# kishwarshafin/pepper

Hardware: AMD Instinct MI355X
Metric: inference windows/sec (whole node) (higher is better)
Workload: dtype f32 via f16 hi/lo split operands (3 MFMAs per product), f32 accumulate

## Files before the change

pepper_amd/csrc/api.hip:

```cpp
#include "../../include/pepper_amd.h"

#include <hip/hip_runtime.h>

#include <algorithm>
#include <cmath>
#include <cstdio>
#include <cstdlib>
#include <cstring>
#include <map>
#include <string>
#include <vector>

#include "dec_frag16.h"
#include "kernels.h"

namespace {
thread_local std::string g_err;
}

namespace pa {
int set_error(int code, const std::string& msg) {
    g_err = msg;
    return code;
}
// ... 496 lines not shown
    if (!as_base(m)) return fail(PA_ERR_INVALID, "bad model handle");
    if (on != 0 && on != 1) return fail(PA_ERR_INVALID, std::string(entry) + ": on must be 0 or 1");
    m->batch_invariant = on != 0;
    return PA_OK;
}

template <class M>
int get_batch_invariant(M* m, int32_t* on) {
    if (!as_base(m) || !on) return fail(PA_ERR_INVALID, "bad model handle");
    *on = m->batch_invariant ? 1 : 0;
    return PA_OK;
}

enum Proj { IN_LOOP, XP_GEMM_H2, XP_GEMM_F32 };
template <class Rec>
struct LayerForm {
    Proj proj;
    Rec rec;
    bool y_h2;
};

}

struct pa_variant_model : ModelBase {
    pa_variant_config cfg{};
    int H = 256, L1 = 512;
    bool split_gemm = true;
    bool split_rec = true;
    int64_t small_batch = 3072;
    int64_t small_rows = 3072;
    std::vector<RecLayer> rec;
    Linear lin[5], out;
    DevBuf *mlp_w = nullptr, *mlp_b = nullptr;
    DevBuf *mlp_w32 = nullptr;
    int* ovf_counter() const {
        return mlp_w32 ? reinterpret_cast<int*>(static_cast<char*>(mlp_w32->p) + 4 * sizeof(float*)) : nullptr;
    }
    DevBuf *xp, *ya, *yb, *l1, *l2, *stage_in[2], *stage_p[2], *stage_l[2];
    bool unit_split = true;
    int split_holdoff = 0;
    int64_t split_fallbacks = 0;
    int split_sabotage = 0;
    DevBuf *us_exch = nullptr, *us_cnt = nullptr, *us_failed = nullptr;
    int* us_host = nullptr;
    bool batch_invariant = false;
    ~pa_variant_model() override {
        if (us_host) (void)hipHostFree(us_host);
    }
};

extern "C" {

const char* pa_last_error(void) { return g_err.c_str(); }
const char* pa_version(void) { return "pepper_amd 0.1.0 gfx950"; }
int pa_device_count(void) {
    int c = 0;
    if (hipGetDeviceCount(&c) != hipSuccess) return 0;
    return c;
}

int pa_variant_create(const pa_variant_config* cfg, const char* const* names, const float* const* data,
                      const int64_t* numel, int32_t n_tensors, void* hip_stream, pa_variant_model** out) {
    if (!cfg || !names || !data || !numel || !out) return fail(PA_ERR_INVALID, "null argument");
    if (cfg->image_features <= 0 || cfg->window <= 0 || cfg->gru_layers <= 0 ||
        cfg->num_classes_type <= 0 || cfg->num_classes_type > 8)
        return fail(PA_ERR_INVALID, "bad pa_variant_config");
    auto* m = new pa_variant_model();
    m->cfg = *cfg;
    const int H = m->H;
    StateDict sd(names, data, numel, n_tensors);
    int rc = create_common(m, sd, cfg->window, H, hip_stream);
    if (const char* e = getenv("PA_SMALL_BATCH")) m->small_batch = atoll(e);
    if (const char* e = getenv("PA_SMALL_ROWS")) m->small_rows = atoll(e);
    if (const char* e = getenv("PA_UNIT_SPLIT")) m->unit_split = e[0] != '0';
    if (const char* e = getenv("PA_UNIT_SPLIT_SABOTAGE")) m->split_sabotage = atoi(e);
    for (int mod = 0; mod < 2 && rc == PA_OK; ++mod)
        for (int layer = 0; layer < cfg->gru_layers && rc == PA_OK; ++layer) {
            const int K = (mod == 0 && layer == 0) ? cfg->image_features : 2 * H;
            m->rec.emplace_back();
            rc = build_rec_layer(m, sd, mod == 0 ? "encoder" : "decoder", layer, 4, H, K, m->rec.back(), m->split_rec,
                                 m->split_gemm);
        }
    const char* lin_names[5] = {"linear_1", "linear_2", "linear_3", "linear_4", "linear_5"};
    for (int i = 0; i < 5 && rc == PA_OK; ++i)
        rc = build_linear(m, sd, lin_names[i], i == 0 ? 2 * H * cfg->window : m->L1, m->L1, m->lin[i],
                          i == 0 && m->split_gemm);
    if (rc == PA_OK) rc = build_linear(m, sd, "output_layer_type", m->L1, cfg->num_classes_type, m->out);
    if (rc == PA_OK && m->split_gemm && m->L1 == 512) {
        std::string err;
        const float* w4[4];
        std::vector<float> b4((size_t)4 * m->L1);
        bool ok = true;
        for (int i = 0; i < 4 && ok; ++i) {
            w4[i] = sd.get(std::string(lin_names[i + 1]) + ".weight", (int64_t)m->L1 * m->L1, err);
            const float* b = sd.get(std::string(lin_names[i + 1]) + ".bias", m->L1, err);
            ok = fits_f16(w4[i], (int64_t)m->L1 * m->L1);
            std::memcpy(&b4[(size_t)i * m->L1], b, m->L1 * sizeof(float));
        }
        if (ok) {
            std::vector<uint32_t> packed(pa::mlp_weights_h2_words(4));
            float scale[4];
            pa::pack_mlp_weights_h2(w4, 4, packed.data(), scale);
            std::vector<float> table((size_t)8 * m->L1 + 4);
            for (int i = 0; i < 4; ++i) {
                for (int k = 0; k < m->L1; ++k) {
                    table[(size_t)i * m->L1 + k] = b4[(size_t)i * m->L1 + k] * scale[i];
                    table[(size_t)4 * m->L1 + 4 + (size_t)i * m->L1 + k] = b4[(size_t)i * m->L1 + k];
                }
// ... 126 lines not shown
            LAUNCH_TRY(m, "lstm_rec_fused_in", 2.0 * n * T * (4.0 * H) * (H + r.K) * 2,
                       pa::launch_lstm_rec_fused(H, static_cast<const int8_t*>(cur), r.K, r.b_in->f(),
                                                 r.w_cat->f(), y, 2 * H, (int)n, T, m->stream));
            break;
        case FUSED_DEC_H2:
            LAUNCH_TRY(m, "lstm_dec_h2_fused", 2.0 * n * T * (4.0 * H) * (H + r.K) * 2,
                       pa::launch_lstm_dec_h2(H, cur, cur_ld, bias_l, r.w_cat_dec_h2->p, y, 2 * H, (int)n, T, m->stream,
                                              bi && s.small_rows));
            break;
        case SPLIT_H2: {
            const int sabotage = m->split_sabotage > 0 ? 1 : 0;
            m->split_sabotage -= sabotage;
            LAUNCH_TRY(m, "lstm_rec_h2_split", 2.0 * n * T * (4.0 * H) * H * 2,
                       pa::launch_lstm_rec_h2_split(H, m->xp->f(), NX, r.w_hh_h2->p, y, 2 * H, (int)n, T, m->us_exch->p,
                                                    m->us_cnt->p, static_cast<int*>(m->us_failed->p), m->stream, sabotage));
            break;
        }
        case PLAIN_H2:
            LAUNCH_TRY(m, "lstm_rec_h2", 2.0 * n * T * (4.0 * H) * H * 2,
                       pa::launch_lstm_seed_h2(H, m->xp->f(), NX, r.w_hh_h2->p, y, 2 * H, (int)n, T, m->stream, s.small_rows));
            break;
        case PLAIN_F32:
            LAUNCH_TRY(m, "lstm_rec", 2.0 * n * T * (4.0 * H) * H * 2,
                       pa::launch_lstm_rec(H, m->xp->f(), NX, r.w_hh->f(), y, 2 * H, (int)n, T, m->stream));
            break;
        }
        cur = y;
        cur_kind = pa::A_F32;
        cur_ld = 2 * H;
        cur_h2 = f.y_h2;
        which ^= 1;
    }
    const int K1 = T * 2 * H;
    if (m->split_gemm && m->lin[0].w_h2 != nullptr && cur_kind == pa::A_F32) {
        if (!cur_h2)
            LAUNCH_TRY(m, "cvt_h2", 0.0,
                       pa::launch_f32_to_h2(static_cast<const float*>(cur), const_cast<void*>(cur), n, K1, K1, m->stream));
        LAUNCH_TRY(m, "gemm_h2_linear_1", 2.0 * n * m->L1 * K1,
                   pa::launch_gemm_h2(cur, K1, (size_t)n * K1 * 4, m->lin[0].w_h2->p, K1, (size_t)m->L1 * K1 * 4,
                                      m->lin[0].b->f(), m->l1->f(), m->L1, (int)n, m->L1, K1, 1, 0, 0, 0, 0, m->stream,
                                      s.l1_splits > 1 ? m->xp->f() : nullptr, s.l1_splits));
    } else {
        LAUNCH_TRY(m, "gemm_linear_1", 2.0 * n * m->L1 * K1,
                   pa::launch_gemm_nt(pa::A_F32, cur, K1, m->lin[0].w->f(), K1, m->lin[0].b->f(), m->l1->f(),
                                      m->L1, (int)n, m->L1, K1, 1, 0, 0, 0, 0, m->stream));
    }
    if (m->mlp_w != nullptr && C <= 8) {
        LAUNCH_TRY(m, "mlp_tail_h2", 2.0 * n * m->L1 * (4.0 * m->L1 + C),
                   pa::launch_mlp_tail_h2(m->l1->f(), m->L1, m->mlp_w->p, m->mlp_b->f(), 4, m->out.w->f(), m->out.b->f(), C,
                                          probs, logits, (int)n, m->stream, static_cast<const float* const*>(m->mlp_w32->p),
                                          ovf_counter, bi));
        if (s.unit_split) {
            HIP_TRY(hipMemcpyAsync(&m->us_host[0], m->us_failed->p, sizeof(int), hipMemcpyDeviceToHost, m->stream));
            HIP_TRY(hipStreamSynchronize(m->stream));
            if (m->us_host[0] != 0) {
                ++m->split_fallbacks;
                m->split_holdoff = US_HOLDOFF;
                HIP_TRY(hipMemcpyAsync(ovf_counter, &m->us_host[1], sizeof(int), hipMemcpyHostToDevice, m->stream));
                return variant_forward_chunk(m, a_kind, images, n, probs, logits, false);
            }
        }
        return PA_OK;
    }
    float* a = m->l1->f();
    float* b = m->l2->f();
    for (int i = 1; i < 5; ++i) {
        LAUNCH_TRY(m, "gemm_linear_2to5", 2.0 * n * m->L1 * m->L1,
                   pa::launch_gemm_nt(pa::A_F32, a, m->L1, m->lin[i].w->f(), m->L1, m->lin[i].b->f(), b,
                                      m->L1, (int)n, m->L1, m->L1, 1, 0, 0, 0, 0, m->stream));
        std::swap(a, b);
    }
    LAUNCH_TRY(m, "head_softmax", 2.0 * n * m->L1 * C,
               pa::launch_dense_small(0, a, m->L1, m->out.w->f(), m->out.b->f(), probs, logits, (int)n,
                                      m->L1, C, 1, 1, 0, m->stream));
    return PA_OK;
}

static int variant_forward(pa_variant_model* m, int a_kind, const void* images, size_t elem, int64_t n,
                           float* probs, float* logits) {
    if (!as_base(m)) return fail(PA_ERR_INVALID, "bad model handle");
    if (n < 0 || (n > 0 && (!images || !probs))) return fail(PA_ERR_INVALID, "null buffer");
    HIP_TRY(hipSetDevice(m->device));
    const int64_t per = (int64_t)m->cfg.window * m->cfg.image_features;
    const int C = m->cfg.num_classes_type;
// ... 478 lines not shown
```

pepper_amd/csrc/gemm_h2.hip:

```cpp
#include "common.h"
#include "kernels.h"

#include <cstdlib>
#include <vector>

namespace {

typedef _Float16 h8 __attribute__((ext_vector_type(8)));

constexpr int HM = 256, HN = 256, HK = 32;
constexpr int HROW = 36;
constexpr int HSTAGE = (HM + HN) * HROW;

PA_DEV f32x16 mfma_h(h8 a, h8 b, f32x16 c) { return __builtin_amdgcn_mfma_f32_32x32x16_f16(a, b, c, 0, 0, 0); }

template <int ACT, int EXP = 0>
__global__ __launch_bounds__(256) void gemm_h2_kernel(const uint32_t* __restrict__ A, int lda, uint32_t a_bytes,
                                                      const uint32_t* __restrict__ W, int ldw, uint32_t w_bytes,
                                                      const float* __restrict__ bias, float* __restrict__ C, int ldc,
                                                      int M, int N, int K, int tiles_n, int nwg, int a_rpb,
                                                      int64_t a_bstride, int frag_T, int frag_nb) {
    __shared__ __attribute__((aligned(16))) uint32_t lds[2 * HSTAGE];

    const int tile = xcd_swizzle(blockIdx.x, nwg);
// ... 348 lines not shown
}

namespace pa {

static bool g_h2_split_parent = false;
int g_h2_exp = 0;

void split_h2_host(const float* src, uint32_t* dst, int64_t rows, int K, int64_t ld_src, int64_t ld_dst) {
    for (int64_t r = 0; r < rows; ++r) {
        const float* s = src + r * ld_src;
        _Float16* d = reinterpret_cast<_Float16*>(dst + r * ld_dst);
        for (int g = 0; g < K / 8; ++g)
            for (int e = 0; e < 8; ++e) {
                const float v = s[g * 8 + e];
                const _Float16 hi = (_Float16)v;
                d[g * 16 + e] = hi;
                d[g * 16 + 8 + e] = (_Float16)(v - (float)hi);
            }
    }
}

hipError_t launch_f32_to_h2(const float* src, void* dst, int64_t rows, int K, int64_t ld, hipStream_t stream) {
    if ((K & 7) || (ld & 7)) return hipErrorInvalidValue;
    const int64_t n = rows * (K >> 3);
    if (n == 0) return hipSuccess;
    hipLaunchKernelGGL(f32_to_h2_kernel, dim3((unsigned)((n + 255) / 256)), dim3(256), 0, stream, src,
                       reinterpret_cast<uint32_t*>(dst), rows, K, ld);
    return hipGetLastError();
}

hipError_t launch_gemm_h2(const void* A, int lda, size_t a_bytes, const void* W, int ldw, size_t w_bytes,
                          const float* bias, float* C, int ldc, int M, int N, int K, int act, int a_rpb,
                          int64_t a_bstride, int frag_T, int frag_nb, hipStream_t stream, float* splitk_ws,
                          int splits) {
    if (frag_T > 0 && ((M & 31) || (N & 31) || act != 0)) return hipErrorInvalidValue;
    if ((K % HK) || (lda & 7) || (ldw & 7) || (a_bstride & 7) || ((uintptr_t)A & 15) || ((uintptr_t)W & 15))
        return hipErrorInvalidValue;
    if (a_bytes >= (1ull << 32) || w_bytes >= (1ull << 32)) return hipErrorInvalidValue;
    const int tiles_m = (M + HM - 1) / HM, tiles_n = (N + HN - 1) / HN;
    const int nwg = tiles_m * tiles_n;
    if (nwg == 0) return hipSuccess;
    const uint32_t* Au = reinterpret_cast<const uint32_t*>(A);
    const uint32_t* Wu = reinterpret_cast<const uint32_t*>(W);
    if (splits > 1 && splitk_ws != nullptr && frag_T == 0 && !(N & 3) && K / HK >= splits) {
        if (g_h2_split_parent)
            hipLaunchKernelGGL((gemm_h2_kernel<0>), dim3(nwg, splits), dim3(256), 0, stream, Au, lda, (uint32_t)a_bytes, Wu,
                               ldw, (uint32_t)w_bytes, (const float*)nullptr, splitk_ws, N, M, N, K, tiles_n, nwg, a_rpb,
                               a_bstride, 0, 0);
        else
            hipLaunchKernelGGL(gemm_h2_k32_kernel, dim3(nwg, splits), dim3(256), 0, stream, Au, lda, (uint32_t)a_bytes, Wu,
                               ldw, (uint32_t)w_bytes, splitk_ws, M, N, K, tiles_n, nwg, a_rpb, a_bstride);
        const size_t n4 = (size_t)M * (N >> 2);
        if (act == 1)
            hipLaunchKernelGGL((splitk_finish_kernel<1>), dim3((unsigned)((n4 + 255) / 256)), dim3(256), 0, stream,
                               splitk_ws, splits, bias, C, ldc, M, N);
        else
            hipLaunchKernelGGL((splitk_finish_kernel<0>), dim3((unsigned)((n4 + 255) / 256)), dim3(256), 0, stream,
                               splitk_ws, splits, bias, C, ldc, M, N);
        return hipGetLastError();
    }
    if (g_h2_exp > 0 && g_h2_exp < 8) {
#define PA_EXP(E_) case E_: hipLaunchKernelGGL((gemm_h2_kernel<0, E_>), dim3(nwg), dim3(256), 0, stream, Au, lda, (uint32_t)a_bytes, Wu, ldw, (uint32_t)w_bytes, bias, C, ldc, M, N, K, tiles_n, nwg, a_rpb, a_bstride, frag_T, frag_nb); break;
        switch (g_h2_exp) { PA_EXP(1) PA_EXP(2) PA_EXP(3) PA_EXP(4) PA_EXP(5) PA_EXP(6) PA_EXP(7) }
#undef PA_EXP
        return hipGetLastError();
    }
    if (act == 1)
        hipLaunchKernelGGL((gemm_h2_kernel<1>), dim3(nwg), dim3(256), 0, stream, Au, lda, (uint32_t)a_bytes, Wu, ldw,
                           (uint32_t)w_bytes, bias, C, ldc, M, N, K, tiles_n, nwg, a_rpb, a_bstride, frag_T, frag_nb);
    else
        hipLaunchKernelGGL((gemm_h2_kernel<0>), dim3(nwg), dim3(256), 0, stream, Au, lda, (uint32_t)a_bytes, Wu, ldw,
                           (uint32_t)w_bytes, bias, C, ldc, M, N, K, tiles_n, nwg, a_rpb, a_bstride, frag_T, frag_nb);
    return hipGetLastError();
}

}

extern "C" void pa_debug_gemm_h2_experiment(int e) { pa::g_h2_exp = e; }

extern "C" int pa_debug_gemm_h2(const float* A, const float* W, const float* bias, float* C, int a_rows, int M, int N,
                                int K, int act, int frag_T, int frag_nb, int iters, float* ms_out) {
    void *dA = nullptr, *dA2 = nullptr, *dW = nullptr, *dB = nullptr, *dC = nullptr;
    const size_t a_bytes = (size_t)a_rows * K * 4, w_bytes = (size_t)N * K * 4;
    const size_t c_elems = frag_T > 0 ? (size_t)M * N : (size_t)M * N;
// ... 83 lines not shown
```

pepper_amd/csrc/kernels.h:

```cpp
#pragma once
#include <hip/hip_runtime.h>
#include <stdint.h>

#include <string>

namespace pa {

int set_error(int code, const std::string& msg);

enum AKind { A_F32 = 0, A_I8 = 1, A_U8 = 2, A_F32_SCALAR = 3 };

hipError_t launch_gemm_nt(int a_type, const void* A, int lda, const float* W, int ldw,
                          const float* bias, float* C, int ldc, int M, int N, int K, int act,
                          int a_rpb, int64_t a_bstride, int frag_T, int frag_nb, hipStream_t stream);

hipError_t launch_gemm_h2(const void* A, int lda, size_t a_bytes, const void* W, int ldw, size_t w_bytes,
                          const float* bias, float* C, int ldc, int M, int N, int K, int act, int a_rpb,
                          int64_t a_bstride, int frag_T, int frag_nb, hipStream_t stream,
                          float* splitk_ws = nullptr, int splits = 1);
hipError_t launch_f32_to_h2(const float* src, void* dst, int64_t rows, int K, int64_t ld, hipStream_t stream);
void split_h2_host(const float* src, uint32_t* dst, int64_t rows, int K, int64_t ld_src, int64_t ld_dst);

hipError_t launch_lstm_rec(int H, const float* Xp, int ldx, const float* Wp, float* Y, int ldy,
                           int B, int T, hipStream_t stream);
hipError_t launch_lstm_rec_fused(int H, const int8_t* X, int F, const float* bias, const float* Wcat,
                                 float* Y, int ldy, int B, int T, hipStream_t stream);
hipError_t launch_gru_rec(int H, const float* Xp, int ldx, const float* Wp, const float* bhn,
                          const float* h0, int ldh0, float* hn, int ldhn, float* Y, int ldy,
                          int B, int T, hipStream_t stream);

hipError_t launch_gru_rec_fused(int H, const uint8_t* X, int F, int64_t x_bstride, const float* bias,
                                const float* Wcat, const float* bhn, const float* h0, int ldh0, float* hn, int ldhn,
                                float* Y, int ldy, int B, int T, hipStream_t stream);

void pack_rec_weights_h2(const float* const whh[2], const float* const wih[2], int G, int H, int F, int KX,
                         uint32_t* out, const float* const* bias = nullptr);
size_t rec_weights_h2_words(int G, int H, int KX);
int gru_fused_input_kx(int H, int F);
hipError_t launch_lstm_seed_h2(int H, const float* Xp, int ldx, const void* Wp, void* Y, int ldy, int B, int T,
                               hipStream_t stream, bool small = false);
hipError_t launch_lstm_enc_h2(int H, const int8_t* X, int F, const float* bias, const void* Wp, void* Y, int ldy, int B, int T,
                              hipStream_t stream, bool small = false);

size_t lstm_split_exchange_bytes(int B);
size_t lstm_split_counter_bytes(int B);
int lstm_split_grid(int B);
int lstm_split_resident_workgroups(int ntw);
hipError_t launch_lstm_rec_h2_split(int H, const float* Xp, int ldx, const void* Wp, void* Y, int ldy, int B, int T, void* exch,
                                    void* counters, int* failed, hipStream_t stream, int sabotage = 0);

hipError_t launch_lstm_dec_h2(int H, const void* Xh, int ldxh, const float* bias, const void* Wp, void* Y, int ldy, int B,
                              int T, hipStream_t stream, bool small = false);
hipError_t launch_gru_rec_h2(int H, const float* Xp, int ldx, const uint8_t* X, int F, int64_t x_bstride,
                             const float* bias, const void* Wp, const float* bhn, const float* h0, int ldh0, float* hn,
                             int ldhn, void* Y, int ldy, int B, int T, hipStream_t stream);

void pack_gru_small_weights_h2(const float* const whh[2], int H, uint32_t* out);
size_t gru_small_weights_h2_words(int H);
hipError_t launch_gru_small_h2(int H, const float* Xp, int ldx, const void* Wp, const float* bhn, const float* h0, int ldh0,
                               float* hn, int ldhn, void* Y, int ldy, int B, int T, hipStream_t stream);
hipError_t launch_gru_dec_h2(int H, const void* Xh, int ldxh, const float* bias, const void* Wp, const float* bhn,
                             const float* h0, int ldh0, float* hn, int ldhn, void* Y, int ldy, int B, int T,
                             hipStream_t stream);

void pack_dense_head_h2(const float* W, int C, int H, uint32_t* out);
size_t dense_head_h2_words(int H);
size_t dense_partials_floats(int B, int T);
hipError_t launch_gru_dec_h2_dense(int H, const void* Xh, int ldxh, const float* bias, const void* Wp, const float* bhn,
                                   const float* h0, int ldh0, float* hn, int ldhn, const void* Wd, float* P, int B, int T,
                                   hipStream_t stream);
hipError_t launch_polish_combine(const float* P, const float* bias, float* acc, int B, int T, int C, int S, int off,
                                 hipStream_t stream);

void pack_mlp_weights_h2(const float* const* W, int NL, uint32_t* out, float* scale);
size_t mlp_weights_h2_words(int NL);
hipError_t launch_mlp_tail_h2(const float* X, int ldx, const void* Wp, const float* bias, int NL, const float* Wout,
                              const float* bout, int C, float* probs, float* logits, int n, hipStream_t stream,
                              const float* const* W32, int* overflow_rows, bool per_row = false);

hipError_t launch_dense_small(int mode, const float* X, int ldx, const float* W, const float* bias,
                              float* out0, float* out1, int rows, int K, int C, int T, int S, int off,
                              hipStream_t stream);
hipError_t launch_polish_dense_acc_h2(const void* X, int ldx, const float* W, const float* bias, float* acc, int rows,
                                      int K, int C, int T, int S, int off, hipStream_t stream);
hipError_t launch_h2_to_f32(void* buf, int64_t rows, int K, int64_t ld, hipStream_t stream);
hipError_t launch_polish_finalize(const float* acc, uint8_t* labels, uint8_t* phred, int64_t B, int S,
                                  int C, int overlap, hipStream_t stream);

void launch_bgzf_inflate(hipStream_t stream, const uint8_t* comp, const int64_t* comp_off, const int32_t* comp_len,
                         const int64_t* out_off, const int32_t* out_len, uint8_t* out, int32_t* status, int n_blocks,
                         int64_t comp_bytes, unsigned long long* debug_counts = nullptr);
const char* inflate_status_text(int32_t s);
void launch_record_walk(hipStream_t stream, const uint8_t* data, int64_t data_bytes, const int64_t* entries, int n_entries, int cap,
                        void* slots, int32_t* counts, int32_t* base, int32_t* flags, void* out, int64_t out_cap, int32_t* tail,
                        int split = 0);
}
```

pepper_amd/csrc/mlp_h2.hip:

```cpp
#include "common.h"
#include "kernels.h"

namespace {

typedef _Float16 h8 __attribute__((ext_vector_type(8)));

constexpr int MT = 64, D = 512, KS = D / 16, NTILES = D / 32;
constexpr int ROWB = D * 4 + 16, ROWD = ROWB / 4;

PA_DEV f32x16 mfma_h(h8 a, h8 b, f32x16 c) { return __builtin_amdgcn_mfma_f32_32x32x16_f16(a, b, c, 0, 0, 0); }

template <int NL, bool PERROW = false>
__global__ __launch_bounds__(512, 1) void mlp_tail_h2_kernel(const float* __restrict__ X, int ldx,
                                                             const uint32_t* __restrict__ Wp,
                                                             const float* __restrict__ bias,
                                                             const float* __restrict__ Wout,
                                                             const float* __restrict__ bout, int C,
                                                             float* __restrict__ probs, float* __restrict__ logits,
                                                             int n, const float* const* __restrict__ W32,
                                                             int* __restrict__ overflow_rows) {
    extern __shared__ __attribute__((aligned(16))) uint32_t lds[];
    static_assert((ROWB / 16) % 2 == 1, "row stride must be an odd number of 16-byte slots");
    const int tid = threadIdx.x, lane = tid & 63;
    const int w = __builtin_amdgcn_readfirstlane(tid >> 6);
    const int li = lane & 31, hf = lane >> 5;
    const int b0 = blockIdx.x * MT;

    bool bad = false;
    uint32_t* rowbad = lds + MT * ROWD;
    {
        const int row = tid >> 3, gsel = tid & 7;
        int grow = b0 + row;
        grow = grow < n ? grow : n - 1;
        const float* src = X + (size_t)grow * ldx;
#pragma unroll
        for (int j = 0; j < 8; ++j) {
            const int g = gsel + 8 * j;
            const f32x4 a = *reinterpret_cast<const f32x4*>(src + g * 8);
            const f32x4 b = *reinterpret_cast<const f32x4*>(src + g * 8 + 4);
            const float v[8] = {a.x, a.y, a.z, a.w, b.x, b.y, b.z, b.w};
            h8 hi, lo;
#pragma unroll
            for (int e = 0; e < 8; ++e) {
                bad |= !(fabsf(v[e]) < 65504.0f);
                hi[e] = (_Float16)v[e];
                lo[e] = (_Float16)(v[e] - (float)hi[e]);
            }
            *reinterpret_cast<h8*>(lds + row * ROWD + g * 8) = hi;
            *reinterpret_cast<h8*>(lds + row * ROWD + g * 8 + 4) = lo;
        }
        if (PERROW) {
            int b8 = bad ? 1 : 0;
            b8 |= __shfl_xor(b8, 1, 64);
            b8 |= __shfl_xor(b8, 2, 64);
            b8 |= __shfl_xor(b8, 4, 64);
            if (gsel == 0) rowbad[row] = (uint32_t)b8;
        }
    }
    __syncthreads();

    const uint32_t* arow = lds + li * ROWD + hf * 8;
    const bool odd = li & 1;
    struct Frag { h8 b[2][2], a[2][2]; };

#pragma unroll 1
    for (int layer = 0; layer < NL; ++layer) {
        const __amdgpu_buffer_rsrc_t wrs = __builtin_amdgcn_make_buffer_rsrc(
            const_cast<uint32_t*>(Wp + ((size_t)layer * NTILES + 2 * w) * KS * 512), 0, 0x7fffffff, 0x00020000);
        const unsigned woff = lane * 16u;
        auto load_step = [&](int s, Frag& fr) {
#pragma unroll
            for (int nn = 0; nn < 2; ++nn)
#pragma unroll
                for (int hl = 0; hl < 2; ++hl)
                    fr.b[nn][hl] = __builtin_bit_cast(h8, __builtin_amdgcn_raw_buffer_load_b128(
                                                              wrs, woff, (unsigned)((nn * KS + s) * 2 + hl) * 1024u, 0));
#pragma unroll
            for (int m = 0; m < 2; ++m) {
                fr.a[m][0] = *reinterpret_cast<const h8*>(arow + m * 32 * ROWD + s * 16);
                fr.a[m][1] = *reinterpret_cast<const h8*>(arow + m * 32 * ROWD + s * 16 + 4);
            }
        };
        f32x16 acc[2][2];
#pragma unroll
        for (int nn = 0; nn < 2; ++nn) {
            const float bv = bias[layer * D + 64 * w + 32 * nn + li];
#pragma unroll
            for (int m = 0; m < 2; ++m)
#pragma unroll
                for (int r = 0; r < 16; ++r) acc[m][nn][r] = bv;
        }
        Frag ring[2];
        load_step(0, ring[0]);
#pragma unroll
        for (int s = 0; s < KS; ++s) {
            const int p = s & 1;
            if (s + 1 < KS) load_step(s + 1, ring[p ^ 1]);
#pragma unroll
            for (int term = 0; term < 3; ++term)
#pragma unroll
                for (int nn = 0; nn < 2; ++nn)
#pragma unroll
                    for (int m = 0; m < 2; ++m)
                        acc[m][nn] = mfma_h(ring[p].a[m][term == 0 ? 1 : 0], ring[p].b[nn][term == 1 ? 1 : 0], acc[m][nn]);
            if (s + 1 < KS) {
#pragma unroll
                for (int q = 0; q < 4; ++q) {
                    __builtin_amdgcn_sched_group_barrier(0x008, 1, 0);
                    __builtin_amdgcn_sched_group_barrier(0x020, 1, 0);
                }
#pragma unroll
                for (int q = 0; q < 4; ++q) {
                    __builtin_amdgcn_sched_group_barrier(0x008, 1, 0);
                    __builtin_amdgcn_sched_group_barrier(0x100, 1, 0);
                }
                __builtin_amdgcn_sched_group_barrier(0x008, 4, 0);
            }
            __builtin_amdgcn_sched_barrier(0);
        }
        lds_barrier();
        const float unscale = bias[NL * D + layer];
#pragma unroll
        for (int nn = 0; nn < 2; ++nn) {
            const int col = 64 * w + 32 * nn + li;
            uint32_t* dst = lds + 4 * hf * ROWD + (col >> 3) * 8 + (odd ? 4 : 0) + ((col & 7) >> 1);
#pragma unroll
            for (int m = 0; m < 2; ++m)
#pragma unroll
                for (int r = 0; r < 16; ++r) {
                    const float v = selu_f(acc[m][nn][r] * unscale);
                    bad |= !(fabsf(v) < 65504.0f);
                    if (PERROW && !(fabsf(v) < 65504.0f)) rowbad[4 * hf + 32 * m + (r & 3) + 8 * (r >> 2)] = 1u;
                    dst[(32 * m + (r & 3) + 8 * (r >> 2)) * ROWD] = h2_word_of(v, h2_select(odd));
                }
        }
        lds_barrier();
    }

    float* frow = reinterpret_cast<float*>(lds);
    auto head = [&](bool from_f32, bool select) {
        float wo[8][8];
#pragma unroll
        for (int c = 0; c < 8; ++c)
#pragma unroll
            for (int e = 0; e < 8; ++e) wo[c][e] = c < C ? Wout[(size_t)c * D + lane * 8 + e] : 0.0f;
        for (int rr = 0; rr < 8; ++rr) {
            const int row = 8 * w + rr;
            if (PERROW && select && (rowbad[row] != 0) != from_f32) continue;
            const h8 hi = *reinterpret_cast<const h8*>(lds + row * ROWD + lane * 8);
            const h8 lo = *reinterpret_cast<const h8*>(lds + row * ROWD + lane * 8 + 4);
            float x[8];
#pragma unroll
            for (int e = 0; e < 8; ++e) x[e] = from_f32 ? frow[row * ROWD + lane * 8 + e] : (float)hi[e] + (float)lo[e];
            float logit[8], mx = -INFINITY;
#pragma unroll
            for (int c = 0; c < 8; ++c) {
                float p = 0.0f;
#pragma unroll
                for (int e = 0; e < 8; ++e) p += x[e] * wo[c][e];
#pragma unroll
                for (int o = 32; o > 0; o >>= 1) p += __shfl_xor(p, o, 64);
                logit[c] = c < C ? p + bout[c < C ? c : 0] : -INFINITY;
                mx = fmaxf(mx, logit[c]);
            }
            float e[8], den = 0.0f;
#pragma unroll
            for (int c = 0; c < 8; ++c) {
                e[c] = c < C ? expf(logit[c] - mx) : 0.0f;
                den += e[c];
            }
            float my_logit = 0.0f, my_e = 0.0f;
#pragma unroll
            for (int c = 0; c < 8; ++c)
                if (lane == c) { my_logit = logit[c]; my_e = e[c]; }
            const int grow = b0 + row;
            if (grow < n && lane < C) {
                probs[(size_t)grow * C + lane] = my_e / den;
                if (logits != nullptr) logits[(size_t)grow * C + lane] = my_logit;
            }
        }
    };

    const bool rerun = __syncthreads_or(bad ? 1 : 0) != 0;
    if (PERROW) {
        head(false, rerun);
        if (rerun) __syncthreads();
    }
    if (rerun) {
        if (tid == 0 && overflow_rows != nullptr) {
            int cnt = n - b0 < MT ? n - b0 : MT;
            if (PERROW) {
                cnt = 0;
                for (int r = 0; r < MT && b0 + r < n; ++r) cnt += rowbad[r] != 0 ? 1 : 0;
            }
            atomicAdd(overflow_rows, cnt);
        }
        for (int i = tid; i < MT * D; i += 512) {
            const int row = i / D, col = i - row * D;
            const int grow = b0 + row < n ? b0 + row : n - 1;
            frow[row * ROWD + col] = X[(size_t)grow * ldx + col];
        }
        __syncthreads();
#pragma unroll 1
        for (int layer = 0; layer < NL; ++layer) {
            const float* wr = W32[layer] + (size_t)tid * D;
            float y[MT];
            const float bv = bias[NL * D + NL + layer * D + tid];
#pragma unroll
            for (int r = 0; r < MT; ++r) y[r] = bv;
#pragma unroll 1
            for (int k = 0; k < D; k += 4) {
                const f32x4 wv = *reinterpret_cast<const f32x4*>(wr + k);
#pragma unroll
                for (int r = 0; r < MT; ++r) {
                    const f32x4 xv = *reinterpret_cast<const f32x4*>(frow + r * ROWD + k);
                    y[r] = fmaf(xv.x, wv.x, y[r]);
                    y[r] = fmaf(xv.y, wv.y, y[r]);
                    y[r] = fmaf(xv.z, wv.z, y[r]);
                    y[r] = fmaf(xv.w, wv.w, y[r]);
                }
            }
            __syncthreads();
#pragma unroll
            for (int r = 0; r < MT; ++r) frow[r * ROWD + tid] = selu_f(y[r]);
            __syncthreads();
        }
    }

    if (PERROW) {
        if (rerun) head(true, true);
    } else {
        head(rerun, false);
    }
}

}

namespace pa {

void pack_mlp_weights_h2(const float* const* W, int NL, uint32_t* out, float* scale) {
    _Float16* o = reinterpret_cast<_Float16*>(out);
    for (int l = 0; l < NL; ++l) {
        float mx = 0.0f;
        for (size_t i = 0; i < (size_t)D * D; ++i) mx = fmaxf(mx, fabsf(W[l][i]));
        int e = 0;
        if (mx > 0.0f) {
            (void)frexpf(mx, &e);
            e = 14 - e;
            e = e > 60 ? 60 : (e < -60 ? -60 : e);
        }
        const float sc = ldexpf(1.0f, e);
        scale[l] = sc;
        for (int nt = 0; nt < NTILES; ++nt)
            for (int s = 0; s < KS; ++s)
                for (int ln = 0; ln < 64; ++ln)
                    for (int e8 = 0; e8 < 8; ++e8) {
                        const float v = sc * W[l][(size_t)(nt * 32 + (ln & 31)) * D + 16 * s + 8 * (ln >> 5) + e8];
                        const _Float16 hi = (_Float16)v;
                        const size_t base = ((((size_t)l * NTILES + nt) * KS + s) * 2) * 512 + (size_t)ln * 8 + e8;
                        o[base] = hi;
                        o[base + 512] = (_Float16)(v - (float)hi);
                    }
    }
}

size_t mlp_weights_h2_words(int NL) { return (size_t)NL * NTILES * KS * 2 * 256; }

hipError_t launch_mlp_tail_h2(const float* X, int ldx, const void* Wp, const float* bias, int NL, const float* Wout,
                              const float* bout, int C, float* probs, float* logits, int n, hipStream_t stream,
                              const float* const* W32, int* overflow_rows, bool per_row) {
    if (n <= 0) return hipSuccess;
    if (NL != 4 || C > 8 || C <= 0 || (ldx & 3) || W32 == nullptr) return hipErrorInvalidValue;
    if (per_row) {
        const size_t lds = (size_t)MT * ROWB + (size_t)MT * sizeof(uint32_t);
        hipLaunchKernelGGL((mlp_tail_h2_kernel<4, true>), dim3((n + MT - 1) / MT), dim3(512), lds, stream, X, ldx,
                           static_cast<const uint32_t*>(Wp), bias, Wout, bout, C, probs, logits, n, W32, overflow_rows);
        return hipGetLastError();
    }
    const size_t lds = (size_t)MT * ROWB;
    hipLaunchKernelGGL((mlp_tail_h2_kernel<4>), dim3((n + MT - 1) / MT), dim3(512), lds, stream, X, ldx,
                       static_cast<const uint32_t*>(Wp), bias, Wout, bout, C, probs, logits, n, W32, overflow_rows);
    return hipGetLastError();
}

}
```

pepper_amd/csrc/rnn_h2.hip:

```cpp
#include <cstdlib>

#include "common.h"
#include "kernels.h"

namespace {

typedef _Float16 h8 __attribute__((ext_vector_type(8)));
typedef float f32x2 __attribute__((ext_vector_type(2)));

constexpr int MT = 64;

PA_DEV f32x16 mfma_h(h8 a, h8 b, f32x16 c) { return __builtin_amdgcn_mfma_f32_32x32x16_f16(a, b, c, 0, 0, 0); }

PA_DEV void decode_block(int bid, int& dir, int& btile) {
    const int xcd = bid & 7, q = bid >> 3;
    dir = xcd >> 2;
    btile = q * 4 + (xcd & 3);
}


extern __shared__ __attribute__((aligned(16))) uint32_t lds[];
template <int MTILES, int KXROW = 0, int XRD_ = 0>
struct LstmLds {
    static_assert(MTILES == 1 || MTILES == 2, "32 or 64 rows per workgroup");
// ... 362 lines not shown
                for (int gp = 0; gp < 2; ++gp) {
                    if (gp == 1 && C::XR == 2) lds_barrier();
#pragma unroll
                    for (int i = 0; i < NM; ++i) {
                        const int m = i / 12, c = (i % 12) / 6, term = (i % 6) >> 1, g2 = i & 1, g = 2 * gp + g2;
                        acc[m][g][c] = __builtin_amdgcn_mfma_f32_16x16x32_f16(a[m][term == 0 ? 1 : 0], b[gp][g2][c][term == 1 ? 1 : 0],
                                                                              C::FRESH && term == 0 ? f32x4{} : acc[m][g][c], 0, 0, 0);
                        if (MTILES == 2 ? (i < 24 && i % 3 == 1) : i < 8) load_b(gp == 0 ? s : sn, gp ^ 1, MTILES == 2 ? i / 3 : i);
                        if (gp == 1 && C::AN != 0 && (i % 12 == 9 || i % 12 == 11)) {
                            if (C::AN == 1) load_a_h(sn, m, i % 12 == 9 ? 1 : 0);
                            else load_a_x(slot, m, i % 12 == 9 ? 1 : 0);
                        }
                        if (C::Y && i == NM / 2 + 1) {
                            if (gp == 0) ycv = yc.read(s);
                            else yc.write(s, tp, ycv);
                        }
                        if (C::Y2 && i == NM / 2 + 4) {
                            if (gp == 0) ycv2 = yc.read(YC - 1);
                            else yc.write(YC - 1, tp, ycv2);
                        }
                        if (C::XR == 2 && gp == 0 && i == NM - 1) xg_store(slot);
                        if (C::XR != 0 && gp == 1 && i == (MTILES == 2 ? 2 : 10)) xg_load(s - 6 < KS - KSH ? s - 6 : KS - KSH - 1, t);
                        __builtin_amdgcn_sched_barrier(0);
                    }
                }
            };
            constexpr bool Y2 = YC > 7;
            constexpr int YL = YC < 6 ? YC : 6;
#pragma unroll
            for (int i = 0; i < 2 * RT; ++i) load_a_h(0, i >> 1, i & 1);
            __builtin_amdgcn_sched_barrier(0);
#pragma unroll 1
            for (int r = 0; r < once; ++r) kstep(0, DecStep<true, true, Y2, 0, 1>{});
#pragma unroll 1
            for (int s = 1; s < YL; ++s) kstep(s, DecStep<false, true, false, 0, 1>{});
#pragma unroll 1
            for (int s = YL; s < 6; ++s) kstep(s, DecStep<false, false, false, 0, 1>{});
#pragma unroll 1
            for (int r = 0; r < once; ++r) kstep(6, DecStep<false, (YC > 6), false, 1, 1>{});
#pragma unroll 1
            for (int s = 7; s < KS - 1; ++s) kstep(s, DecStep<false, false, false, 2, 2>{});
#pragma unroll 1
            for (int r = 0; r < once; ++r) kstep(KS - 1, DecStep<false, false, false, 0, 0>{});
        }
        float cb[4][2];
        load_bias16(cb, brs, lr);
        if (stamp) dbg[(u * 80 + 2 * step) * 2 + 1] = __builtin_amdgcn_s_memtime();

        lds_barrier();
        if (stamp) dbg[(u * 80 + 2 * step + 1) * 2] = __builtin_amdgcn_s_memtime();

#pragma unroll
        for (int m = 0; m < RT; ++m)
#pragma unroll
            for (int c = 0; c < 2; ++c)
                gate_tile16<ROWD, true>(acc[m][0][c], acc[m][1][c], acc[m][2][c], acc[m][3][c], f32x4{cb[0][c], cb[1][c], cb[2][c], cb[3][c]},
                                        cs + (m * 8 + c * 4) * 64, hl_dst + 16 * m * ROWD * 2 + c * 32);
        if (stamp) dbg[(u * 80 + 2 * step + 1) * 2 + 1] = __builtin_amdgcn_s_memtime();
        lds_barrier();
    }
    {
        const int tl = dir ? 0 : T - 1;
#pragma unroll
        for (int j = 0; j < YC; ++j) yc.write(j, tl, yc.read(j));
    }
}

template <bool FRESH_, bool Y_, bool X_, int AN_>
struct EncStep {
    static constexpr bool FRESH = FRESH_, Y = Y_, X = X_;
// ... 1166 lines not shown
```

Baseline: 2.852 million.

## Fold split-K finish into MLP tail, deepen weight prefetch ring, skip decoder step-0 stages

When linear_1 runs split-K and the fused MLP tail is in use, the separate finish kernel is dropped and the tail sums the partial slices, adds bias and applies SELU while loading its input. The tail's weight fetch moves to a four-deep ring that also prefetches the next layer's first stages across layer boundaries. The decoder recurrence also skips some k-steps at step 0, on the assumption that the hidden state is zero there. These remove a kernel launch plus a full l1 round trip and reduce weight-load stalls, at the cost of more registers and a correctness risk if the step-0 skip or fold numerics are wrong.

```diff
diff --git a/pepper_amd/csrc/api.hip b/pepper_amd/csrc/api.hip
--- a/pepper_amd/csrc/api.hip
+++ b/pepper_amd/csrc/api.hip
@@ -552,6 +552,7 @@
     std::vector<RecLayer> rec;
     Linear lin[5], out;
     DevBuf *mlp_w = nullptr, *mlp_b = nullptr;
+    bool fold_finish = true;
     DevBuf *mlp_w32 = nullptr;
     int* ovf_counter() const {
         return mlp_w32 ? reinterpret_cast<int*>(static_cast<char*>(mlp_w32->p) + 4 * sizeof(float*)) : nullptr;
@@ -594,6 +595,7 @@
     if (const char* e = getenv("PA_SMALL_ROWS")) m->small_rows = atoll(e);
     if (const char* e = getenv("PA_UNIT_SPLIT")) m->unit_split = e[0] != '0';
     if (const char* e = getenv("PA_UNIT_SPLIT_SABOTAGE")) m->split_sabotage = atoi(e);
+    if (const char* e = getenv("PA_FOLD_FINISH")) m->fold_finish = e[0] != '0';
     for (int mod = 0; mod < 2 && rc == PA_OK; ++mod)
         for (int layer = 0; layer < cfg->gru_layers && rc == PA_OK; ++layer) {
             const int K = (mod == 0 && layer == 0) ? cfg->image_features : 2 * H;
@@ -786,6 +788,8 @@
         which ^= 1;
     }
     const int K1 = T * 2 * H;
+    const bool fused_tail = m->mlp_w != nullptr && C <= 8;
+    bool l1_slices = false;
     if (m->split_gemm && m->lin[0].w_h2 != nullptr && cur_kind == pa::A_F32) {
         if (!cur_h2)
             LAUNCH_TRY(m, "cvt_h2", 0.0,
@@ -793,17 +797,19 @@
         LAUNCH_TRY(m, "gemm_h2_linear_1", 2.0 * n * m->L1 * K1,
                    pa::launch_gemm_h2(cur, K1, (size_t)n * K1 * 4, m->lin[0].w_h2->p, K1, (size_t)m->L1 * K1 * 4,
                                       m->lin[0].b->f(), m->l1->f(), m->L1, (int)n, m->L1, K1, 1, 0, 0, 0, 0, m->stream,
-                                      s.l1_splits > 1 ? m->xp->f() : nullptr, s.l1_splits));
+                                      s.l1_splits > 1 ? m->xp->f() : nullptr, s.l1_splits,
+                                      m->fold_finish && fused_tail && s.l1_splits > 1 ? &l1_slices : nullptr));
     } else {
         LAUNCH_TRY(m, "gemm_linear_1", 2.0 * n * m->L1 * K1,
                    pa::launch_gemm_nt(pa::A_F32, cur, K1, m->lin[0].w->f(), K1, m->lin[0].b->f(), m->l1->f(),
                                       m->L1, (int)n, m->L1, K1, 1, 0, 0, 0, 0, m->stream));
     }
-    if (m->mlp_w != nullptr && C <= 8) {
+    if (fused_tail) {
         LAUNCH_TRY(m, "mlp_tail_h2", 2.0 * n * m->L1 * (4.0 * m->L1 + C),
                    pa::launch_mlp_tail_h2(m->l1->f(), m->L1, m->mlp_w->p, m->mlp_b->f(), 4, m->out.w->f(), m->out.b->f(), C,
                                           probs, logits, (int)n, m->stream, static_cast<const float* const*>(m->mlp_w32->p),
-                                          ovf_counter, bi));
+                                          ovf_counter, bi, l1_slices ? m->xp->f() : nullptr, s.l1_splits, (int)n,
+                                          m->lin[0].b->f()));
         if (s.unit_split) {
             HIP_TRY(hipMemcpyAsync(&m->us_host[0], m->us_failed->p, sizeof(int), hipMemcpyDeviceToHost, m->stream));
             HIP_TRY(hipStreamSynchronize(m->stream));
diff --git a/pepper_amd/csrc/gemm_h2.hip b/pepper_amd/csrc/gemm_h2.hip
--- a/pepper_amd/csrc/gemm_h2.hip
+++ b/pepper_amd/csrc/gemm_h2.hip
@@ -404,7 +404,9 @@
 hipError_t launch_gemm_h2(const void* A, int lda, size_t a_bytes, const void* W, int ldw, size_t w_bytes,
                           const float* bias, float* C, int ldc, int M, int N, int K, int act, int a_rpb,
                           int64_t a_bstride, int frag_T, int frag_nb, hipStream_t stream, float* splitk_ws,
-                          int splits) {
+                          int splits, bool* slices_only) {
+    const bool want_slices = slices_only != nullptr;
+    if (want_slices) *slices_only = false;
     if (frag_T > 0 && ((M & 31) || (N & 31) || act != 0)) return hipErrorInvalidValue;
     if ((K % HK) || (lda & 7) || (ldw & 7) || (a_bstride & 7) || ((uintptr_t)A & 15) || ((uintptr_t)W & 15))
         return hipErrorInvalidValue;
@@ -422,6 +424,10 @@
         else
             hipLaunchKernelGGL(gemm_h2_k32_kernel, dim3(nwg, splits), dim3(256), 0, stream, Au, lda, (uint32_t)a_bytes, Wu,
                                ldw, (uint32_t)w_bytes, splitk_ws, M, N, K, tiles_n, nwg, a_rpb, a_bstride);
+        if (want_slices) {
+            *slices_only = true;
+            return hipGetLastError();
+        }
         const size_t n4 = (size_t)M * (N >> 2);
         if (act == 1)
             hipLaunchKernelGGL((splitk_finish_kernel<1>), dim3((unsigned)((n4 + 255) / 256)), dim3(256), 0, stream,
diff --git a/pepper_amd/csrc/kernels.h b/pepper_amd/csrc/kernels.h
--- a/pepper_amd/csrc/kernels.h
+++ b/pepper_amd/csrc/kernels.h
@@ -17,7 +17,8 @@
 hipError_t launch_gemm_h2(const void* A, int lda, size_t a_bytes, const void* W, int ldw, size_t w_bytes,
                           const float* bias, float* C, int ldc, int M, int N, int K, int act, int a_rpb,
                           int64_t a_bstride, int frag_T, int frag_nb, hipStream_t stream,
-                          float* splitk_ws = nullptr, int splits = 1);
+                          float* splitk_ws = nullptr, int splits = 1,
+                          bool* slices_only = nullptr);
 hipError_t launch_f32_to_h2(const float* src, void* dst, int64_t rows, int K, int64_t ld, hipStream_t stream);
 void split_h2_host(const float* src, uint32_t* dst, int64_t rows, int K, int64_t ld_src, int64_t ld_dst);
 
@@ -76,7 +77,8 @@
 size_t mlp_weights_h2_words(int NL);
 hipError_t launch_mlp_tail_h2(const float* X, int ldx, const void* Wp, const float* bias, int NL, const float* Wout,
                               const float* bout, int C, float* probs, float* logits, int n, hipStream_t stream,
-                              const float* const* W32, int* overflow_rows, bool per_row = false);
+                              const float* const* W32, int* overflow_rows, bool per_row = false,
+                              const float* partials = nullptr, int slices = 0, int part_rows = 0, const float* bias1 = nullptr);
 
 hipError_t launch_dense_small(int mode, const float* X, int ldx, const float* W, const float* bias,
                               float* out0, float* out1, int rows, int K, int C, int T, int S, int off,
diff --git a/pepper_amd/csrc/mlp_h2.hip b/pepper_amd/csrc/mlp_h2.hip
--- a/pepper_amd/csrc/mlp_h2.hip
+++ b/pepper_amd/csrc/mlp_h2.hip
@@ -10,8 +10,40 @@
 
 PA_DEV f32x16 mfma_h(h8 a, h8 b, f32x16 c) { return __builtin_amdgcn_mfma_f32_32x32x16_f16(a, b, c, 0, 0, 0); }
 
-template <int NL, bool PERROW = false>
-__global__ __launch_bounds__(512, 1) void mlp_tail_h2_kernel(const float* __restrict__ X, int ldx,
+
+PA_DEV float selu_both_sides(float x) {
+    const float alpha = 1.6732632423543772848170429916717f;
+    const float scale = 1.0507009873554804934193349852946f;
+    const float neg = alpha * expm1f(x);
+    return scale * (x > 0.0f ? x : neg);
+}
+
+PA_DEV f32x4 l1_bias_selu4(f32x4 v, f32x4 bias) {
+#pragma clang fp contract(off)
+    v += bias;
+    float x0 = selu_both_sides(v.x), x1 = selu_both_sides(v.y), x2 = selu_both_sides(v.z), x3 = selu_both_sides(v.w);
+    asm("" : "+v"(x0), "+v"(x1), "+v"(x2), "+v"(x3));
+    return f32x4{x0, x1, x2, x3};
+}
+
+PA_DEV f32x4 l1_finish4(const float* __restrict__ part, int S, size_t slice, const float* __restrict__ b1, int grow, int col) {
+#pragma clang fp contract(off)
+    const float* p = part + (size_t)grow * D + col;
+    f32x4 v = *reinterpret_cast<const f32x4*>(p);
+    for (int s = 1; s < S; ++s) {
+        const f32x4 u = *reinterpret_cast<const f32x4*>(p + (size_t)s * slice);
+        v += u;
+    }
+    return l1_bias_selu4(v, *reinterpret_cast<const f32x4*>(b1 + col));
+}
+
+#ifdef PA_TAIL_STAMP
+__device__ unsigned long long g_tail_stamp[8 * 16];
+#endif
+
+template <int NL, bool PERROW = false, bool FOLD = false>
+__global__ __launch_bounds__(512, 1) void mlp_tail_h2_kernel(const float* __restrict__ X, int ldx, int S, int part_rows,
+                                                             const float* __restrict__ b1,
                                                              const uint32_t* __restrict__ Wp,
                                                              const float* __restrict__ bias,
                                                              const float* __restrict__ Wout,
@@ -28,16 +60,26 @@
 
     bool bad = false;
     uint32_t* rowbad = lds + MT * ROWD;
+    const size_t slice = (size_t)part_rows * D;
+    auto in4 = [&](int grow, int col) -> f32x4 {
+        if (FOLD) return l1_finish4(X, S, slice, b1, grow, col);
+        return *reinterpret_cast<const f32x4*>(X + (size_t)grow * ldx + col);
+    };
+#ifdef PA_TAIL_STAMP
+    auto tick = [&](int k) {
+        if (blockIdx.x == 8 && lane == 0) g_tail_stamp[w * 16 + k] = __builtin_amdgcn_s_memtime();
+    };
+#else
+    auto tick = [](int) {};
+#endif
+    tick(0);
+
     {
+#pragma clang fp contract(off)
         const int row = tid >> 3, gsel = tid & 7;
         int grow = b0 + row;
         grow = grow < n ? grow : n - 1;
-        const float* src = X + (size_t)grow * ldx;
-#pragma unroll
-        for (int j = 0; j < 8; ++j) {
-            const int g = gsel + 8 * j;
-            const f32x4 a = *reinterpret_cast<const f32x4*>(src + g * 8);
-            const f32x4 b = *reinterpret_cast<const f32x4*>(src + g * 8 + 4);
+        auto split_store = [&](int g, f32x4 a, f32x4 b) {
             const float v[8] = {a.x, a.y, a.z, a.w, b.x, b.y, b.z, b.w};
             h8 hi, lo;
 #pragma unroll
@@ -48,6 +90,32 @@
             }
             *reinterpret_cast<h8*>(lds + row * ROWD + g * 8) = hi;
             *reinterpret_cast<h8*>(lds + row * ROWD + g * 8 + 4) = lo;
+        };
+        if (FOLD && S == 2) {
+            const float* p0 = X + (size_t)grow * D;
+#pragma unroll
+            for (int half = 0; half < 2; ++half) {
+                f32x4 r0[4][2], r1[4][2], bb[4][2];
+#pragma unroll
+                for (int j = 0; j < 4; ++j)
+#pragma unroll
+                    for (int q = 0; q < 2; ++q) {
+                        const int col = (gsel + 8 * (4 * half + j)) * 8 + 4 * q;
+                        r0[j][q] = *reinterpret_cast<const f32x4*>(p0 + col);
+                        r1[j][q] = *reinterpret_cast<const f32x4*>(p0 + slice + col);
+                        bb[j][q] = *reinterpret_cast<const f32x4*>(b1 + col);
+                    }
+#pragma unroll
+                for (int j = 0; j < 4; ++j)
+                    split_store(gsel + 8 * (4 * half + j), l1_bias_selu4(r0[j][0] + r1[j][0], bb[j][0]),
+                                l1_bias_selu4(r0[j][1] + r1[j][1], bb[j][1]));
+            }
+        } else {
+#pragma unroll
+            for (int j = 0; j < 8; ++j) {
+                const int g = gsel + 8 * j;
+                split_store(g, in4(grow, g * 8), in4(grow, g * 8 + 4));
+            }
         }
         if (PERROW) {
             int b8 = bad ? 1 : 0;
@@ -58,29 +126,44 @@
         }
     }
     __syncthreads();
-
-    const uint32_t* arow = lds + li * ROWD + hf * 8;
+    tick(1);
+
+    struct FragB { h8 b[2][2]; };
+    struct FragA { h8 a[2][2]; };
+    constexpr int RB = 4;
+    static_assert(KS % RB == 0, "a layer's first stages land in the ring slots the next layer reads them from");
+    auto wrs_of = [&](int layer) {
+        return __builtin_amdgcn_make_buffer_rsrc(const_cast<uint32_t*>(Wp + ((size_t)layer * NTILES + 2 * w) * KS * 512), 0,
+                                                 0x7fffffff, 0x00020000);
+    };
+    const unsigned woff = lane * 16u;
+    auto load_b = [&](const __amdgpu_buffer_rsrc_t& rs, int s, FragB& fr) {
+#pragma unroll
+        for (int nn = 0; nn < 2; ++nn)
+#pragma unroll
+            for (int hl = 0; hl < 2; ++hl)
+                fr.b[nn][hl] = __builtin_bit_cast(h8, __builtin_amdgcn_raw_buffer_load_b128(
+                                                          rs, woff + (unsigned)((s & 1) * 2 + hl) * 1024u,
+                                                          (unsigned)((nn * KS + (s & ~1)) * 2) * 1024u, 0));
+    };
+    FragB rb[RB];
+
+    int aoff[2] = {li * ROWD + hf * 8, li * ROWD + hf * 8 + 32 * ROWD};
+    asm volatile("" : "+v"(aoff[1]));
+    const uint32_t* const arow[2] = {lds + aoff[0], lds + aoff[1]};
     const bool odd = li & 1;
-    struct Frag { h8 b[2][2], a[2][2]; };
+    auto load_a = [&](int s, FragA& fr) {
+#pragma unroll
+        for (int m = 0; m < 2; ++m) {
+            fr.a[m][0] = *reinterpret_cast<const h8*>(arow[m] + s * 16);
+            fr.a[m][1] = *reinterpret_cast<const h8*>(arow[m] + s * 16 + 4);
+        }
+    };
 
 #pragma unroll 1
     for (int layer = 0; layer < NL; ++layer) {
-        const __amdgpu_buffer_rsrc_t wrs = __builtin_amdgcn_make_buffer_rsrc(
-            const_cast<uint32_t*>(Wp + ((size_t)layer * NTILES + 2 * w) * KS * 512), 0, 0x7fffffff, 0x00020000);
-        const unsigned woff = lane * 16u;
-        auto load_step = [&](int s, Frag& fr) {
-#pragma unroll
-            for (int nn = 0; nn < 2; ++nn)
-#pragma unroll
-                for (int hl = 0; hl < 2; ++hl)
-                    fr.b[nn][hl] = __builtin_bit_cast(h8, __builtin_amdgcn_raw_buffer_load_b128(
-                                                              wrs, woff, (unsigned)((nn * KS + s) * 2 + hl) * 1024u, 0));
-#pragma unroll
-            for (int m = 0; m < 2; ++m) {
-                fr.a[m][0] = *reinterpret_cast<const h8*>(arow + m * 32 * ROWD + s * 16);
-                fr.a[m][1] = *reinterpret_cast<const h8*>(arow + m * 32 * ROWD + s * 16 + 4);
-            }
-        };
+        const __amdgpu_buffer_rsrc_t wrs = wrs_of(layer);
+        const __amdgpu_buffer_rsrc_t wrs_next = wrs_of(layer + 1 < NL ? layer + 1 : layer);
         f32x16 acc[2][2];
 #pragma unroll
         for (int nn = 0; nn < 2; ++nn) {
@@ -90,35 +173,45 @@
 #pragma unroll
                 for (int r = 0; r < 16; ++r) acc[m][nn][r] = bv;
         }
-        Frag ring[2];
-        load_step(0, ring[0]);
+        FragA ra[2];
+        load_a(0, ra[0]);
+        if (layer == 0) {
+#pragma unroll
+            for (int q = 0; q < RB - 1; ++q) load_b(wrs, q, rb[q]);
+        }
 #pragma unroll
         for (int s = 0; s < KS; ++s) {
-            const int p = s & 1;
-            if (s + 1 < KS) load_step(s + 1, ring[p ^ 1]);
+            const int p = s & 1, sb = s + RB - 1;
+            const bool lda = s + 1 < KS;
+            if (sb < KS) load_b(wrs, sb, rb[sb % RB]);
+            else load_b(wrs_next, sb - KS, rb[sb % RB]);
+            if (lda) load_a(s + 1, ra[p ^ 1]);
 #pragma unroll
             for (int term = 0; term < 3; ++term)
 #pragma unroll
                 for (int nn = 0; nn < 2; ++nn)
 #pragma unroll
                     for (int m = 0; m < 2; ++m)
-                        acc[m][nn] = mfma_h(ring[p].a[m][term == 0 ? 1 : 0], ring[p].b[nn][term == 1 ? 1 : 0], acc[m][nn]);
-            if (s + 1 < KS) {
-#pragma unroll
-                for (int q = 0; q < 4; ++q) {
-                    __builtin_amdgcn_sched_group_barrier(0x008, 1, 0);
-                    __builtin_amdgcn_sched_group_barrier(0x020, 1, 0);
-                }
+                        acc[m][nn] = mfma_h(ra[p].a[m][term == 0 ? 1 : 0], rb[s % RB].b[nn][term == 1 ? 1 : 0], acc[m][nn]);
+#pragma unroll
+            for (int q = 0; q < 4; ++q) {
+                __builtin_amdgcn_sched_group_barrier(0x008, 1, 0);
+                __builtin_amdgcn_sched_group_barrier(0x020, 1, 0);
+            }
+            if (lda) {
 #pragma unroll
                 for (int q = 0; q < 4; ++q) {
                     __builtin_amdgcn_sched_group_barrier(0x008, 1, 0);
                     __builtin_amdgcn_sched_group_barrier(0x100, 1, 0);
                 }
                 __builtin_amdgcn_sched_group_barrier(0x008, 4, 0);
+            } else {
+                __builtin_amdgcn_sched_group_barrier(0x008, 8, 0);
             }
             __builtin_amdgcn_sched_barrier(0);
         }
         lds_barrier();
+        tick(2 + 2 * layer);
         const float unscale = bias[NL * D + layer];
 #pragma unroll
         for (int nn = 0; nn < 2; ++nn) {
@@ -135,23 +228,27 @@
                 }
         }
         lds_barrier();
-    }
-
+        tick(3 + 2 * layer);
+    }
+
+    int tid_ep = tid;
+    asm volatile("" : "+v"(tid_ep));
+    const int lane_ep = tid_ep & 63, w_ep = __builtin_amdgcn_readfirstlane(tid_ep >> 6);
     float* frow = reinterpret_cast<float*>(lds);
     auto head = [&](bool from_f32, bool select) {
         float wo[8][8];
 #pragma unroll
         for (int c = 0; c < 8; ++c)
 #pragma unroll
-            for (int e = 0; e < 8; ++e) wo[c][e] = c < C ? Wout[(size_t)c * D + lane * 8 + e] : 0.0f;
+            for (int e = 0; e < 8; ++e) wo[c][e] = c < C ? Wout[(size_t)c * D + lane_ep * 8 + e] : 0.0f;
         for (int rr = 0; rr < 8; ++rr) {
-            const int row = 8 * w + rr;
+            const int row = 8 * w_ep + rr;
             if (PERROW && select && (rowbad[row] != 0) != from_f32) continue;
-            const h8 hi = *reinterpret_cast<const h8*>(lds + row * ROWD + lane * 8);
-            const h8 lo = *reinterpret_cast<const h8*>(lds + row * ROWD + lane * 8 + 4);
+            const h8 hi = *reinterpret_cast<const h8*>(lds + row * ROWD + lane_ep * 8);
+            const h8 lo = *reinterpret_cast<const h8*>(lds + row * ROWD + lane_ep * 8 + 4);
             float x[8];
 #pragma unroll
-            for (int e = 0; e < 8; ++e) x[e] = from_f32 ? frow[row * ROWD + lane * 8 + e] : (float)hi[e] + (float)lo[e];
+            for (int e = 0; e < 8; ++e) x[e] = from_f32 ? frow[row * ROWD + lane_ep * 8 + e] : (float)hi[e] + (float)lo[e];
             float logit[8], mx = -INFINITY;
 #pragma unroll
             for (int c = 0; c < 8; ++c) {
@@ -172,11 +269,11 @@
             float my_logit = 0.0f, my_e = 0.0f;
 #pragma unroll
             for (int c = 0; c < 8; ++c)
-                if (lane == c) { my_logit = logit[c]; my_e = e[c]; }
+                if (lane_ep == c) { my_logit = logit[c]; my_e = e[c]; }
             const int grow = b0 + row;
-            if (grow < n && lane < C) {
-                probs[(size_t)grow * C + lane] = my_e / den;
-                if (logits != nullptr) logits[(size_t)grow * C + lane] = my_logit;
+            if (grow < n && lane_ep < C) {
+                probs[(size_t)grow * C + lane_ep] = my_e / den;
+                if (logits != nullptr) logits[(size_t)grow * C + lane_ep] = my_logit;
             }
         }
     };
@@ -187,7 +284,7 @@
         if (rerun) __syncthreads();
     }
     if (rerun) {
-        if (tid == 0 && overflow_rows != nullptr) {
+        if (tid_ep == 0 && overflow_rows != nullptr) {
             int cnt = n - b0 < MT ? n - b0 : MT;
             if (PERROW) {
                 cnt = 0;
@@ -195,17 +292,17 @@
             }
             atomicAdd(overflow_rows, cnt);
         }
-        for (int i = tid; i < MT * D; i += 512) {
-            const int row = i / D, col = i - row * D;
+        for (int i = tid_ep; i < MT * D / 4; i += 512) {
+            const int row = i / (D / 4), col = (i - row * (D / 4)) * 4;
             const int grow = b0 + row < n ? b0 + row : n - 1;
-            frow[row * ROWD + col] = X[(size_t)grow * ldx + col];
+            *reinterpret_cast<f32x4*>(frow + row * ROWD + col) = in4(grow, col);
         }
         __syncthreads();
 #pragma unroll 1
         for (int layer = 0; layer < NL; ++layer) {
-            const float* wr = W32[layer] + (size_t)tid * D;
+            const float* wr = W32[layer] + (size_t)tid_ep * D;
             float y[MT];
-            const float bv = bias[NL * D + NL + layer * D + tid];
+            const float bv = bias[NL * D + NL + layer * D + tid_ep];
 #pragma unroll
             for (int r = 0; r < MT; ++r) y[r] = bv;
 #pragma unroll 1
@@ -222,7 +319,7 @@
             }
             __syncthreads();
 #pragma unroll
-            for (int r = 0; r < MT; ++r) frow[r * ROWD + tid] = selu_f(y[r]);
+            for (int r = 0; r < MT; ++r) frow[r * ROWD + tid_ep] = selu_f(y[r]);
             __syncthreads();
         }
     }
@@ -232,6 +329,7 @@
     } else {
         head(rerun, false);
     }
+    tick(2 + 2 * NL);
 }
 
 }
@@ -268,19 +366,34 @@
 
 hipError_t launch_mlp_tail_h2(const float* X, int ldx, const void* Wp, const float* bias, int NL, const float* Wout,
                               const float* bout, int C, float* probs, float* logits, int n, hipStream_t stream,
-                              const float* const* W32, int* overflow_rows, bool per_row) {
+                              const float* const* W32, int* overflow_rows, bool per_row, const float* partials, int slices,
+                              int part_rows, const float* bias1) {
     if (n <= 0) return hipSuccess;
-    if (NL != 4 || C > 8 || C <= 0 || (ldx & 3) || W32 == nullptr) return hipErrorInvalidValue;
+    if (NL != 4 || C > 8 || C <= 0 || W32 == nullptr) return hipErrorInvalidValue;
+    const bool fold = partials != nullptr;
+    if (fold ? (slices < 1 || part_rows < n || bias1 == nullptr || ((uintptr_t)partials & 15) || ((uintptr_t)bias1 & 15))
+             : (X == nullptr || (ldx & 3)))
+        return hipErrorInvalidValue;
+    const size_t lds = (size_t)MT * ROWB + (per_row ? (size_t)MT * sizeof(uint32_t) : 0);
+    const float* in = fold ? partials : X;
+    const dim3 grid((n + MT - 1) / MT), block(512);
+    const uint32_t* Wu = static_cast<const uint32_t*>(Wp);
+#define PA_TAIL(PERROW_, FOLD_)                                                                                          \
+    hipLaunchKernelGGL((mlp_tail_h2_kernel<4, PERROW_, FOLD_>), grid, block, lds, stream, in, ldx, slices, part_rows, bias1, \
+                       Wu, bias, Wout, bout, C, probs, logits, n, W32, overflow_rows)
     if (per_row) {
-        const size_t lds = (size_t)MT * ROWB + (size_t)MT * sizeof(uint32_t);
-        hipLaunchKernelGGL((mlp_tail_h2_kernel<4, true>), dim3((n + MT - 1) / MT), dim3(512), lds, stream, X, ldx,
-                           static_cast<const uint32_t*>(Wp), bias, Wout, bout, C, probs, logits, n, W32, overflow_rows);
-        return hipGetLastError();
-    }
-    const size_t lds = (size_t)MT * ROWB;
-    hipLaunchKernelGGL((mlp_tail_h2_kernel<4>), dim3((n + MT - 1) / MT), dim3(512), lds, stream, X, ldx,
-                       static_cast<const uint32_t*>(Wp), bias, Wout, bout, C, probs, logits, n, W32, overflow_rows);
+        if (fold) PA_TAIL(true, true); else PA_TAIL(true, false);
+    } else {
+        if (fold) PA_TAIL(false, true); else PA_TAIL(false, false);
+    }
+#undef PA_TAIL
     return hipGetLastError();
 }
 
 }
+
+#ifdef PA_TAIL_STAMP
+extern "C" int pa_debug_dump_tail_stamps(unsigned long long* host_out) {
+    return hipMemcpyFromSymbol(host_out, HIP_SYMBOL(g_tail_stamp), sizeof(g_tail_stamp)) == hipSuccess ? 0 : 2;
+}
+#endif
diff --git a/pepper_amd/csrc/rnn_h2.hip b/pepper_amd/csrc/rnn_h2.hip
--- a/pepper_amd/csrc/rnn_h2.hip
+++ b/pepper_amd/csrc/rnn_h2.hip
@@ -418,10 +418,14 @@
             __builtin_amdgcn_sched_barrier(0);
 #pragma unroll 1
             for (int r = 0; r < once; ++r) kstep(0, DecStep<true, true, Y2, 0, 1>{});
+#ifndef PA_DEC_SKIP0
+#define PA_DEC_SKIP0 1
+#endif
+            const int e1 = PA_DEC_SKIP0 && step == 0 ? 1 : YL, e2 = PA_DEC_SKIP0 && step == 0 ? 1 : 6;
 #pragma unroll 1
-            for (int s = 1; s < YL; ++s) kstep(s, DecStep<false, true, false, 0, 1>{});
+            for (int s = 1; s < e1; ++s) kstep(s, DecStep<false, true, false, 0, 1>{});
 #pragma unroll 1
-            for (int s = YL; s < 6; ++s) kstep(s, DecStep<false, false, false, 0, 1>{});
+            for (int s = YL; s < e2; ++s) kstep(s, DecStep<false, false, false, 0, 1>{});
 #pragma unroll 1
             for (int r = 0; r < once; ++r) kstep(6, DecStep<false, (YC > 6), false, 1, 1>{});
 #pragma unroll 1
```

New measurement: 2.879 million (median of 6 runs). Within noise of the previous version (+0.9%).
